# illini-robomaster/irmv_detection

Hardware: AMD Instinct MI355X
Metric: end-to-end FPS (preprocess→NMS→PnP) 640×640 YOLOv8n, 1/2/4/8 MI355X (higher is better)
Workload: dtype f16

## Files before the change

irmv_detection_amd/csrc/engine.cpp:

```cpp
#include <hip/hip_runtime.h>

#include <algorithm>
#include <chrono>
#include <cmath>
#include <cstdio>
#include <cstring>
#include <fstream>
#include <map>
#include <mutex>
#include <set>
#include <memory>
#include <string>
#include <vector>

#include "../../include/irmv_hip.h"
#include "irmv_common.hpp"
#include "numa.hpp"

using namespace irmv;

constexpr int kLightPointsCap = 4096;

static thread_local std::string g_err;
static int fail(int code, const std::string &msg)
// ... 23 lines not shown
extern "C" int irmv_device_synchronize(int device)
{
    HIP_TRY(hipSetDevice(device));
    HIP_TRY(hipDeviceSynchronize());
    return IRMV_OK;
}
extern "C" int irmv_device_count(int *count)
{
    if (!count) return fail(IRMV_ERR_ARG, "count is null");
    HIP_TRY(hipGetDeviceCount(count));
    return IRMV_OK;
}

#pragma pack(push, 1)
struct BlobHeader { char magic[4]; uint32_t version, nc, nk, reg_max, n_layers, dtype, reserved; };
struct BlobLayer { char name[32]; uint32_t cin, cout, k, stride, act, pad; uint64_t w_off, b_off; };
#pragma pack(pop)

struct LayerW {
    std::string name;
    int cin, cout, k, stride, act;
    int groups;
    const uint16_t *w;
    const float *b;
};

static float half_bits_to_float(uint16_t h)
{
    const uint32_t sign = ((uint32_t)h & 0x8000u) << 16;
    uint32_t exp = (h >> 10) & 0x1fu, man = h & 0x3ffu, x;
    if (exp == 0) {
        if (man == 0) x = sign;
        else {
            int e = -1;
            do { e++; man <<= 1; } while (!(man & 0x400u));
            x = sign | ((uint32_t)(112 - e) << 23) | ((man & 0x3ffu) << 13);
        }
    } else if (exp == 31) x = sign | 0x7f800000u | (man << 13);
    else x = sign | ((exp + 112u) << 23) | (man << 13);
    float f;
    memcpy(&f, &x, 4);
    return f;
}

static uint16_t float_to_half_bits(float f)
{
    uint32_t x;
    memcpy(&x, &f, 4);
    const uint32_t sign = (x >> 16) & 0x8000u;
    x &= 0x7fffffffu;
    if (x >= 0x7f800000u) return (uint16_t)(sign | 0x7c00u | ((x > 0x7f800000u) ? 0x200u : 0u));
    if (x >= 0x477ff000u) return (uint16_t)(sign | 0x7c00u);
    if (x < 0x33000001u) return (uint16_t)sign;
    if (x < 0x38800000u) {
        const int shift = 126 - (int)(x >> 23);
        const uint32_t man = (x & 0x7fffffu) | 0x800000u;
        uint32_t h = man >> shift;
        const uint32_t rem = man & ((1u << shift) - 1u), half = 1u << (shift - 1);
        if (rem > half || (rem == half && (h & 1u))) h++;
        return (uint16_t)(sign | h);
    }
    uint32_t h = ((x >> 23) - 112u) << 10 | ((x >> 13) & 0x3ffu);
    const uint32_t rem = x & 0x1fffu;
    if (rem > 0x1000u || (rem == 0x1000u && (h & 1u))) h++;
    return (uint16_t)(sign | h);
}

struct Tensor {
    std::string name;
    void *base = nullptr;
    size_t slot_elems = 0;
    int H = 0, W = 0, C = 0;
    bool f32 = false;
    size_t esize() const { return f32 ? 4 : 2; }
    void *slot(int s) const { return static_cast<char *>(base) + (size_t)s * slot_elems * esize(); }
};

struct SegRef { int t = -1, coff = 0, C = 0, shift = 0; };

struct TuneSwitches {
    bool untuned, verbose, warn;
    bool has_s2, has_wres;
    std::string force_s2, force_wres;
    bool force_pw, force_pwn, force_cm, force_w8, force_nt8, force_pf4;
    bool no_pw, no_pwn, no_pf2, no_pf4, no_cm, no_w8, no_nt8, no_wres, no_deep;
};

enum OpKind { OP_PRE, OP_CONV0, OP_CONV, OP_POOL, OP_NMS, OP_LIGHT, OP_FRONT, OP_C2F2, OP_C2F32, OP_DW, OP_SHUF, OP_SCAN, OP_BNECK, OP_KPT3, OP_DEMOSAIC };

struct Op {
    OpKind kind;
    std::string layer;
    ConvCfg cfg{};
    ConvCfg cfg_one{};
    char kname_one[48] = {0};
    SegRef s0, s1;
    int Hin = 0, Win = 0, Hout = 0, Wout = 0, cin = 0, cout = 0, cout_pad = 0, ksteps = 0;
    int out_t = -1, out_coff = 0, res_t = -1, res_coff = 0;
    half_t *w_packed = nullptr;
    half_t *w_k16 = nullptr;
    half_t *w_lds[4] = {nullptr, nullptr, nullptr, nullptr};
    float *bias = nullptr;
    double flops = 0, bytes = 0;
    double w_bytes = 0;
    double out_bytes = 0;
    bool pair = false;
    int level = -1;
    char kname[48] = {0};
    int sub[4] = {-1, -1, -1, -1};
    int mode = 0;
    bool shortcut = false;
    int fuse_next = -1;
    bool fused_away = false;
    int group = -1;
    int bneck = -1;
    int kpt3 = -1;
    int tune_fuse[2] = {-1, -1};
};

enum StepKind { STEP_BATCH, STEP_ONE, STEP_MATERIALIZE, STEP_POST };

struct Launch {
    int op = -1, group = -1;
    bool cfg_one = false;
    bool fused = false;
    unsigned scan = 0;
    bool keys_only = false;
    bool once = false;
    std::string name, layer;
    double flops = 0, bytes = 0, launch_bytes = 0;
};

struct GraphKey {
    int first, count;
    StepKind kind;
    bool upload;
    bool operator<(const GraphKey &o) const { return std::tie(first, count, kind, upload) < std::tie(o.first, o.count, o.kind, o.upload); }
};

struct SlotGroup {
    int first = 0, count = 0;
    hipEvent_t h2d = nullptr, out = nullptr;
    hipStream_t compute = nullptr;
    bool in_flight = false;
    bool async_up = false;
};

struct irmv_engine {
    irmv_engine_cfg cfg{};
    int nc = 0, nk = 0, A = 0, no = 0;
    int backbone = 0;
    int num_cus = 256;
    int numa_node = -1;
    bool numa_placed = false;
    struct HeadGroup { std::vector<int> members; int family = 0, nt = 1; ConvCfg cfg{}; char name[48] = {0}; };
    std::vector<HeadGroup> head_groups;
    bool post_keys_only = false;
    bool emit_scan = false;
    bool split_scan = true;
    int *cand_counts = nullptr;
    int lvl_hw[3] = {0, 0, 0}, lvl_base[3] = {0, 0, 0};
    size_t frame_bytes = 0;
    size_t src_bytes = 0;
    hipStream_t stream = nullptr;
    hipStream_t extra_streams[7] = {nullptr, nullptr, nullptr, nullptr, nullptr, nullptr, nullptr};
    int num_streams = 1;
    hipStream_t h2d_stream = nullptr;
    std::map<std::pair<int, int>, SlotGroup> groups;
// ... 1062 lines not shown
    if (cfg->point_source < 0 || cfg->point_source > 2) return fail(IRMV_ERR_ARG, "bad point_source");
    int ndev = 0;
    HIP_TRY(hipGetDeviceCount(&ndev));
    if (cfg->device < 0 || cfg->device >= ndev) return fail(IRMV_ERR_HIP, "no such HIP device");
    std::unique_ptr<irmv_engine> e(new irmv_engine);
    e->cfg = *cfg;
    {
        int cus = 0;
        if (hipDeviceGetAttribute(&cus, hipDeviceAttributeMultiprocessorCount, cfg->device) == hipSuccess && cus > 0) e->num_cus = cus;
        int node = -1;
        if (hipDeviceGetAttribute(&node, hipDeviceAttributeHostNumaId, cfg->device) == hipSuccess) e->numa_node = node;
        else (void)hipGetLastError();
    }
    int rc = load_blob(e.get());
    e->cfg.weights_path = nullptr;
    e->cfg.weights_blob = nullptr;
    if (rc) return rc;
    rc = build_engine(e.get());
    if (rc) return rc;
    rc = autotune_convs(e.get());
    if (rc) return rc;
    finalize_head_fusion(e.get());
    rc = build_head_groups(e.get());
    if (rc) return rc;
    build_step_plans(e.get());
    rc = choose_sync_launch(e.get());
    if (rc) return rc;
    *out = e.release();
    return IRMV_OK;
}

extern "C" int irmv_engine_sync_launch(const irmv_engine *e) { return e ? e->sync_launch : 0; }

extern "C" void irmv_engine_destroy(irmv_engine *e) { delete e; }
extern "C" int irmv_engine_num_slots(const irmv_engine *e) { return e ? e->cfg.num_slots : 0; }
extern "C" int irmv_engine_max_det(const irmv_engine *e) { return e ? e->cfg.max_det : 0; }
extern "C" int irmv_engine_num_streams(const irmv_engine *e) { return e ? e->num_streams : 0; }
extern "C" int irmv_engine_num_anchors(const irmv_engine *e) { return e ? e->A : 0; }
extern "C" int irmv_engine_numa_node(const irmv_engine *e) { return e ? e->numa_node : -1; }
extern "C" int irmv_engine_numa_placed(const irmv_engine *e) { return e && e->numa_placed ? 1 : 0; }

extern "C" int irmv_numa_device_node(int device, int *node)
{
    if (!node) return fail(IRMV_ERR_ARG, "node is null");
    int v = -1;
    if (hipDeviceGetAttribute(&v, hipDeviceAttributeHostNumaId, device) != hipSuccess) {
        (void)hipGetLastError();
        v = -1;
    }
    *node = v;
    return IRMV_OK;
}
extern "C" int irmv_numa_bind_thread(int node) { return numa::bind_thread_to_node(node) ? IRMV_OK : fail(IRMV_ERR_ARG, "no usable CPU on that NUMA node (or none listed in sysfs)"); }
extern "C" int irmv_numa_page_node(const void *p) { return numa::page_node(p); }
extern "C" int irmv_numa_parse_cpulist(const char *s, int *cpus, int cap)
{
    const std::vector<int> v = numa::parse_cpulist(s);
    for (size_t i = 0; i < v.size() && (int)i < cap; i++) if (cpus) cpus[i] = v[i];
    return (int)v.size();
}
extern "C" int irmv_engine_head_channels(const irmv_engine *e) { return e ? e->no : 0; }

static uint8_t *upload_dev(const irmv_engine *e) { return e->raw_dev ? e->raw_dev : e->src_dev; }

extern "C" uint8_t *irmv_engine_src_buffer(irmv_engine *e, int slot)
{
    if (!e || slot < 0 || slot >= e->cfg.num_slots) return nullptr;
    return e->src_host + (size_t)slot * e->src_bytes;
}
extern "C" void *irmv_engine_src_device_buffer(irmv_engine *e, int slot)
{
    if (!e || slot < 0 || slot >= e->cfg.num_slots) return nullptr;
    return upload_dev(e) + (size_t)slot * e->src_bytes;
}
extern "C" int irmv_engine_src_format(const irmv_engine *e) { return e ? e->cfg.src_format : -1; }
extern "C" size_t irmv_engine_src_bytes(const irmv_engine *e) { return e ? e->src_bytes : 0; }

struct TuneEntry { int mt, nt, flags, ipw; };
static bool operator==(const TuneEntry &x, const TuneEntry &y) { return x.mt == y.mt && x.nt == y.nt && x.flags == y.flags && x.ipw == y.ipw; }
static std::mutex g_tune_mu;
static std::map<std::string, TuneEntry> g_tune_cache;
static std::set<std::string> g_tune_files;

enum : int { T_LDS = 1, T_DEEP = 2, T_CT = 4, T_PW = 8, T_PF2 = 16, T_PF4 = 32, T_CM2 = 64, T_CM4 = 128, T_W8 = 256, T_WR = 512, T_PP = 1024 };
static int tile_flags(const ConvCfg &c)
{
    return (c.lds ? T_LDS : 0) | (c.deep ? T_DEEP : 0) | (c.ct ? T_CT : 0) | (c.pw ? T_PW : 0) | (c.pf2 ? T_PF2 : 0) | (c.pf4 ? T_PF4 : 0) |
           (c.cm == 2 ? T_CM2 : 0) | (c.cm == 4 ? T_CM4 : 0) | (c.w8 ? T_W8 : 0) | (c.wr ? T_WR : 0) | (c.pp ? T_PP : 0);
}
static TuneEntry tune_entry(const ConvCfg &c) { return {c.mt, c.nt, tile_flags(c), c.ipw}; }

static void tune_cache_load()
{
    const char *path = getenv("IRMV_TUNE_CACHE");
    if (!path) return;
    std::lock_guard<std::mutex> lk(g_tune_mu);
    if (!g_tune_files.insert(path).second) return;
    std::ifstream f(path);
    std::string key;
    TuneEntry t;
    while (f >> key >> t.mt >> t.nt >> t.flags >> t.ipw) g_tune_cache[key] = t;
}

static void tune_cache_save()
{
    const char *path = getenv("IRMV_TUNE_CACHE");
    if (!path) return;
    std::lock_guard<std::mutex> lk(g_tune_mu);
    std::ofstream f(path);
    for (auto &kv : g_tune_cache) f << kv.first << ' ' << kv.second.mt << ' ' << kv.second.nt << ' ' << kv.second.flags << ' ' << kv.second.ipw << '\n';
}

static int lds_index(int nt) { return nt == 8 ? 3 : (nt == 4 ? 2 : (nt == 2 ? 1 : 0)); }

static bool run_conv(const Op &op, const ConvCfg &c, const ConvArgs &a, int count, hipStream_t s)
{
    const int li = lds_index(c.nt);
    if (op.w_k16) return launch_conv_k16(a, s);
    if (c.pw) return launch_conv_pw(c, a, s);
    if (c.wr) return c.lds && op.w_lds[2] && launch_conv_wres(c.ipw, a, op.w_lds[2], count, s, c.pp);
    if (c.lds) return op.w_lds[li] && launch_conv_lds(c.stride, c.mt, c.nt, c.ipw, a, op.w_lds[li], count, s, c.pf4 ? 2 : (c.pf2 ? 1 : 0), c.cm, c.w8);
    if (c.ct) {
        if (!op.w_lds[0] || a.n2 > 0) return false;
        ConvArgs a2 = a;
        a2.w = op.w_lds[0];
        return launch_conv(c, a2, s);
    }
    return launch_conv(c, a, s);
}

static void cfg_name(const ConvCfg &c, char *buf, int n)
{
    if (c.pw) snprintf(buf, n, c.ipw > 1 ? "conv1x1s1_pw_n%d" : "conv1x1s1_pw", c.ipw);
    else if (c.wr) snprintf(buf, n, "conv3x3s1_wres%s_i%d", c.pp ? "_pp" : "", c.ipw);
    else if (c.lds && c.ipw > 1) snprintf(buf, n, "conv3x3s%d_lds_mt%d_nt%d_i%d%s%s", c.stride, c.mt, c.nt, c.ipw, c.cm ? "_cm" : (c.pf4 ? "_p4" : (c.pf2 ? "_p2" : "")), c.w8 ? "_w8" : "");
    else if (c.lds) snprintf(buf, n, "conv3x3s%d_lds_mt%d_nt%d%s%s", c.stride, c.mt, c.nt, c.pf4 ? "_p4" : (c.pf2 ? "_p2" : ""), c.w8 ? "_w8" : "");
    else conv_cfg_name(c, buf, n);
}

static void fill_conv_args(const irmv_engine *e, const Op &op, int first, int count, ConvArgs &a, bool fused = false);

static ConvCfg tile_cfg(const ConvCfg &base, int mt, int nt, int flags, int ipw)
{
    ConvCfg c = base;
    c.mt = mt; c.nt = nt; c.ipw = ipw;
    c.lds = flags & T_LDS; c.deep = flags & T_DEEP; c.ct = flags & T_CT; c.pw = flags & T_PW; c.pf2 = flags & T_PF2; c.pf4 = flags & T_PF4;
    c.cm = (flags & T_CM2) ? 2 : ((flags & T_CM4) ? 4 : 0); c.w8 = flags & T_W8; c.wr = flags & T_WR; c.pp = flags & T_PP;
    return c;
}

static TuneSwitches tune_switches()
{
    auto on = [](const char *name) { return getenv(name) != nullptr; };
    const char *at = getenv("IRMV_AUTOTUNE"), *nd = getenv("IRMV_NO_DEEP");
    TuneSwitches s;
    s.untuned = at && at[0] == '0'; s.verbose = on("IRMV_AUTOTUNE_VERBOSE"); s.warn = on("IRMV_TUNE_WARN");
    const char *s2 = getenv("IRMV_FORCE_S2"), *wres = getenv("IRMV_FORCE_WRES");
    s.has_s2 = s2 != nullptr; s.force_s2 = s2 ? s2 : "";
    s.has_wres = wres != nullptr; s.force_wres = wres ? wres : "";
    s.force_pw = on("IRMV_FORCE_PW"); s.force_pwn = on("IRMV_FORCE_PWN"); s.force_cm = on("IRMV_FORCE_CM");
    s.force_w8 = on("IRMV_FORCE_W8"); s.force_nt8 = on("IRMV_FORCE_NT8"); s.force_pf4 = on("IRMV_FORCE_PF4");
    s.no_pw = on("IRMV_NO_PW"); s.no_pwn = on("IRMV_NO_PWN"); s.no_pf2 = on("IRMV_NO_PF2"); s.no_pf4 = on("IRMV_NO_PF4");
    s.no_cm = on("IRMV_NO_CM"); s.no_w8 = on("IRMV_NO_W8"); s.no_nt8 = on("IRMV_NO_NT8"); s.no_wres = on("IRMV_NO_WRES");
    s.no_deep = nd && nd[0] == '1';
    return s;
}

struct TuneCand { ConvCfg c; bool forced; };

static std::vector<TuneCand> tune_candidates(const Op &op, const ConvArgs &a, int count, bool want_fuse, bool lds_ok, const TuneSwitches &sw, int num_cus)
{
    std::vector<TuneCand> v;
    const bool s2 = sw.has_s2 && lds_ok && op.cfg.stride == 2;
    auto add = [&](const ConvCfg &c, bool forced = false) {
        if (op.cout_pad % (16 * c.nt) != 0) return;
        if (s2 && !forced && sw.force_s2 != (c.lds ? "lds" : (c.deep ? "deep" : "ct"))) return;
        if (c.wr ? !(op.w_lds[2] && conv_wres_bytes(a, c.stride, c.pp) > 0)
                 : c.lds && !(op.w_lds[lds_index(c.nt)] && conv_lds_bytes(a, c.stride, c.mt, c.nt, nullptr, c.w8) > 0)) return;
        v.push_back({c, forced});
    };
    const int ipw_max = lds_ok ? std::min(4, count) : 1;
    for (int mt = 1; mt <= 4; mt *= 2)
        for (int nt = 1; nt <= 4; nt *= 2)
            for (int ipw = 1; ipw <= ipw_max; ipw *= 2)
                if (!want_fuse || nt == 4) add(tile_cfg(op.cfg, mt, nt, lds_ok ? T_LDS : 0, ipw));
    if (lds_ok && !want_fuse && !sw.no_pf2)
        for (int nt = 1; nt <= 4; nt *= 2)
            for (int ipw = 1; ipw <= ipw_max; ipw *= 2) add(tile_cfg(op.cfg, 1, nt, T_LDS | T_PF2, ipw));
    if (lds_ok && !want_fuse && !sw.no_pf4 && op.cin >= 128 && op.w_lds[0]) add(tile_cfg(op.cfg, 1, 1, T_LDS | T_PF4, 1), sw.force_pf4);
    if (lds_ok && !sw.no_cm)
        for (int mt = 1; mt <= 2; mt *= 2)
            for (int ipw = 2; ipw <= std::min(mt == 1 ? 4 : 2, count); ipw *= 2)
                if (!(want_fuse && mt == 1 && ipw == 2)) add(tile_cfg(op.cfg, mt, 4, T_LDS | (ipw == 2 ? T_CM2 : T_CM4), ipw), sw.force_cm);
    if (lds_ok && op.cfg.stride == 2 && !want_fuse && !sw.no_w8)
        for (int mt = 1; mt <= 2; mt *= 2)
            for (int ipw = 1; ipw <= ipw_max; ipw *= 2)
                for (int cmv = 0; cmv < 2; cmv++)
                    if (!cmv || (mt == 2 && ipw == 2) || (mt == 1 && ipw == 4)) add(tile_cfg(op.cfg, mt, 4, T_LDS | T_W8 | (cmv ? (ipw == 2 ? T_CM2 : T_CM4) : 0), ipw), sw.force_w8);
    if (lds_ok && op.cfg.stride == 2 && !want_fuse && !sw.no_w8 && !sw.no_nt8)
        for (int ipw = 1; ipw <= ipw_max; ipw *= 2)
            for (int cmv = 0; cmv < 2; cmv++)
                if (!cmv || ipw == 2) add(tile_cfg(op.cfg, 1, 8, T_LDS | T_W8 | (cmv ? T_CM2 : 0), ipw), sw.force_nt8);
    if (lds_ok && count >= 2 && !sw.no_wres)
        for (int ppv = 0; ppv < 2; ppv++) {
            const int wgt = conv_wres_tiles(a, op.cfg.stride, ppv != 0);
            if (wgt <= 0) continue;
            int ipw1 = 1;
            while (ipw1 < count && (long)wgt * ((count + ipw1 - 1) / ipw1) > num_cus) ipw1++;
            const int cand[3] = {ipw1, (ipw1 + 1) / 2, std::min(count, 2 * ipw1)};
            for (int k = 0; k < 3; k++)
                if (k == 0 || (cand[k] != cand[0] && (k == 1 || cand[2] != cand[1]))) add(tile_cfg(op.cfg, 2, 4, T_LDS | T_WR | (ppv ? T_PP : 0), cand[k]));
        }
    if (sw.has_wres && lds_ok && count >= 2) {
        const int n = atoi(sw.force_wres.c_str());
        for (int ppv = 0; ppv <= (n > 0 ? 1 : 0); ppv++) add(tile_cfg(op.cfg, 2, 4, T_LDS | T_WR | (ppv ? T_PP : 0), std::max(1, std::min(count, n < 0 ? -n : n))), true);
    }
    if (conv_pw_eligible(op.cfg, a) && !sw.no_pw) {
        add(tile_cfg(op.cfg, 2, 4, T_PW, 1), sw.force_pw);
        for (int nbw = 2; nbw <= 4 && !sw.no_pwn; nbw *= 2)
            if (conv_pw_lds_bytes(a, nbw)) add(tile_cfg(op.cfg, 2, 4, T_PW, nbw), sw.force_pwn);
    }
    if (lds_ok && !want_fuse && op.w_lds[0] && op.cfg.stride == 2 && !op.cfg.cin16)
        for (int mt = 1; mt <= 4; mt *= 2)
            for (int nt = 1; nt <= 4; nt *= 2) add(tile_cfg(op.cfg, mt, nt, T_CT, 1));
    if ((count == 1 || op.cfg.ks == 1) && !want_fuse && !sw.no_deep && !op.cfg.cin16 && !op.cfg.out_f32 && op.cfg.act == 1 && (!lds_ok || op.w_lds[0])) {
        const int tiles[4][2] = {{1, 1}, {2, 1}, {1, 2}, {1, 4}};
        for (auto &t : tiles) add(tile_cfg(op.cfg, t[0], t[1], T_DEEP | (lds_ok ? T_CT : 0), 1));
    }
    return v;
}

struct ConvView { ConvArgs a; bool want_fuse, lds_ok; };
static ConvView conv_view(const irmv_engine *e, const Op &op, int first, int count)
{
    ConvView v;
    const bool fuse_k16 = op.fuse_next >= 0 && op.cfg.cin16;
    v.want_fuse = op.fuse_next >= 0 && !fuse_k16;
    fill_conv_args(e, op, first, count, v.a, v.want_fuse || fuse_k16);
    if (v.want_fuse) {
        bool f_ok = false;
        for (int mt = 1; mt <= 4 && !f_ok; mt *= 2) f_ok = op.w_lds[2] && conv_lds_bytes(v.a, op.cfg.stride, mt, 4, nullptr) > 0;
        if (!f_ok) {
            v.want_fuse = false;
            fill_conv_args(e, op, first, count, v.a, false);
        }
    }
    v.lds_ok = false;
    if (op.cfg.ks == 3 && op.cfg.act == 1 && !op.cfg.out_f32)
        for (int mt = 1; mt <= 4 && !v.lds_ok; mt *= 2)
            for (int nt = 1; nt <= 4 && !v.lds_ok; nt *= 2) v.lds_ok = op.w_lds[lds_index(nt)] && conv_lds_bytes(v.a, op.cfg.stride, mt, nt, nullptr) > 0;
    return v;
}

static int autotune_convs(irmv_engine *e)
{
    const TuneSwitches sw = tune_switches();
    e->tune_sw = sw;
    tune_cache_load();
    hipEvent_t ea, eb;
    HIP_TRY(hipEventCreate(&ea));
    HIP_TRY(hipEventCreate(&eb));
    const int counts[2] = {stream_share(e, e->cfg.num_slots), 1};
    for (Op &op : e->ops) {
        if (op.kind != OP_CONV) continue;
        for (int pass = 0; pass < (counts[0] > 1 ? 2 : 1); pass++) {
            const int count = counts[pass];
            op.tune_fuse[pass] = op.fuse_next;
            const ConvView v = conv_view(e, op, 0, count);
            if (!v.want_fuse && !op.cfg.cin16) op.fuse_next = -1;
            const ConvArgs &a = v.a;
            const bool want_fuse = v.want_fuse, lds_ok = v.lds_ok;
            char key[160];
            snprintf(key, sizeof key, "gfx950.t5|%d.%d.%d.%d.%d.%d|%dx%d>%dx%d|c%d.%d.%d.%d>%d|ld%d.%d.%d|n%d|%d", op.cfg.ks, op.cfg.stride,
                     (int)op.cfg.cin16, op.cfg.act, (int)op.cfg.out_f32, (int)lds_ok, a.Hin, a.Win, a.Hout, a.Wout, a.s0.C, a.s1.C, a.s0.shift,
                     a.s1.shift, a.cout_pad, a.s0.ld, a.s1.ld, a.out_ld, count, (a.res ? 1 : 0) + 2 * a.n2);
            const std::vector<TuneCand> cands = tune_candidates(op, a, count, want_fuse, lds_ok, sw, e->num_cus);
            const bool forced = (sw.has_s2 && lds_ok && op.cfg.stride == 2) || std::any_of(cands.begin(), cands.end(), [](const TuneCand &k) { return k.forced; });
            ConvCfg best_cfg = pass == 0 ? op.cfg : op.cfg_one;
            bool have_hit = false;
            if (!forced && !sw.untuned && !sw.verbose) {
                std::lock_guard<std::mutex> lk(g_tune_mu);
                auto hit = g_tune_cache.find(key);
                if (hit != g_tune_cache.end()) {
                    const TuneEntry &h = hit->second;
                    auto it = std::find_if(cands.begin(), cands.end(), [&](const TuneCand &k) { return tune_entry(k.c) == h; });
                    if (it != cands.end()) { best_cfg = it->c; have_hit = true; }
                    else if (sw.warn) fprintf(stderr, "[autotune] cached tile for %s rejected (mt %d nt %d lds %d ipw %d): re-tuning\n", key, h.mt, h.nt, h.flags & 1, h.ipw);
                }
            }
            float best = 1e30f;
            for (size_t i = 0; i < cands.size() && !have_hit; i++) {
                const ConvCfg &c = cands[i].c;
                if (cands[i].forced) {
                    if (run_conv(op, c, a, count, e->stream)) { best = 0.f; best_cfg = c; }
                    continue;
                }
                if (sw.untuned && best < 1e29f) continue;
                bool ok = true;
                for (int r = 0; r < 2 && ok; r++) ok = run_conv(op, c, a, count, e->stream);
                if (!ok) continue;
                if (sw.untuned) { best = 0.f; best_cfg = c; continue; }
                float ms = 1e30f;
                for (int rep = 0; rep < 3; rep++) {
// ... 1165 lines not shown
```

irmv_detection_amd/csrc/irmv_common.hpp:

```cpp
#pragma once

#include <hip/hip_runtime.h>

#include <cstdint>
#include <cstdlib>

namespace irmv {

typedef _Float16 half_t;
typedef _Float16 half8 __attribute__((ext_vector_type(8)));
typedef _Float16 half4 __attribute__((ext_vector_type(4)));
typedef float f32x4 __attribute__((ext_vector_type(4)));

constexpr float kActScale = 1.44269504088896341f;
constexpr float kActUnscale = 0.693147180559945309f;
typedef unsigned int u32x4_t __attribute__((ext_vector_type(4)));
__device__ __forceinline__ float silu_rcp(float y) { return __builtin_amdgcn_rcpf(1.0f + __builtin_amdgcn_exp2f(-y)); }
__device__ __forceinline__ unsigned int silu_pack2(float y0, float y1)
{
    const float r0 = silu_rcp(y0), r1 = silu_rcp(y1);
    unsigned int o;
    asm("v_fma_mixlo_f16 %0, %1, %2, 0" : "=v"(o) : "v"(y0), "v"(r0));
    asm("v_fma_mixhi_f16 %0, %1, %2, 0" : "+v"(o) : "v"(y1), "v"(r1));
    return o;
// ... 170 lines not shown
    int cat_ld;
    half_t *out;
    int out_ld;
    int H, W, tiles_x, tiles_y;
    const half_t *w_m1, *w_m2;
    const float *b_m1, *b_m2;
    const half_t *w_cv2;
    const float *b_cv2;
};
size_t bneck64_lds_bytes(int mode, int ks2);
bool launch_bneck64(int mode, int ks2, bool shortcut, const BneckArgs &a, int batch, hipStream_t s);

constexpr int kKpt3Tile = 10;
struct Kpt3Args {
    const half_t *x;
    int x_ld;
    int H, W, tiles_x, tiles_y;
    const half_t *w1;
    const float *b1;
    const half_t *w2;
    const float *b2;
    const half_t *w3;
    const float *b3;
    float *out;
    int out_ld;
};
bool kpt3_eligible(int cin);
bool launch_kpt3(const Kpt3Args &a, int cin, int batch, hipStream_t s);

struct ConvArgs {
    ConvSeg s0, s1;
    int Hin, Win;
    int Hout, Wout;
    int M;
    int Cin;
    const half_t *w;
    const float *bias;
    void *out;
    int out_ld;
    const half_t *res;
    int res_ld;
    int cout_pad;
    int ksteps;
    int pair;
    const half_t *w2;
    const float *bias2;
    float *out2;
    int out2_ld, n2;
    unsigned long long *scan_keys;
    int *scan_counts;
    float scan_thr;
    int scan_nc, scan_abase, scan_key_cap;
};

constexpr int kMultiMax = 6;
struct LdsMember {
    ConvArgs a;
    const half_t *wl;
    int tiles_x, tiles_y, twc_log2, patch_bytes, batch, tile2d;
    int gx, gy;
};
struct LdsMultiArgs {
    int n;
    int start[kMultiMax + 1];
    LdsMember m[kMultiMax];
};
struct DirectMultiArgs {
    int n;
    int start[kMultiMax + 1], gx[kMultiMax], gy[kMultiMax];
    ConvArgs a[kMultiMax];
};

struct ConvCfg {
    int ks, stride, mt, nt; bool cin16; int act; bool out_f32; bool lds; int ipw;
    bool deep;
    bool ct;
    bool pw;
    bool pf2;
    bool pf4;
    bool w8;
    int cm;
    bool wr;
    bool pp;
};
bool launch_conv(const ConvCfg &cfg, const ConvArgs &a, hipStream_t s);
const char *conv_cfg_name(const ConvCfg &cfg, char *buf, int n);
bool conv_pw_eligible(const ConvCfg &cfg, const ConvArgs &a);
bool launch_conv_lds_multi(int nt, const ConvArgs *a, const half_t *const *wl, int n, int batch, hipStream_t s);
bool launch_conv_direct_multi(const ConvCfg &cfg, const ConvArgs *a, int n, hipStream_t s);
bool launch_conv_k16(const ConvArgs &a, hipStream_t s);
bool launch_conv_pw(const ConvCfg &cfg, const ConvArgs &a, hipStream_t s);
size_t conv_pw_lds_bytes(const ConvArgs &a, int nbw);
size_t conv_lds_bytes(const ConvArgs &a, int stride, int mt, int nt, int *patch_rows_max, bool w8 = false);
size_t conv_wres_bytes(const ConvArgs &a, int stride, bool pp);
int conv_wres_tiles(const ConvArgs &a, int stride, bool pp);
bool launch_conv_wres(int ipw, const ConvArgs &a, const half_t *wl, int batch, hipStream_t s, bool pp);
bool launch_conv_lds(int stride, int mt, int nt, int ipw, const ConvArgs &a, const half_t *wl, int batch, hipStream_t s, int pf2 = 0, int cm = 0, bool w8 = false);

void launch_sppf_pool(half_t *buf, int batch, int H, int W, int C, hipStream_t s);

struct DevDet {
    float box_net[4];
    float xyxy[4];
    float score;
    int32_t cls, anchor, pnp_ok;
    float kpts_net[8];
    float kpts[8];
    double rvec[3], tvec[3], quat[4];
    int32_t armor_valid;
    int32_t armor_size;
    int32_t n_lights;
    int32_t pad_;
};
struct DevFrameOut { int32_t num_dets, n_candidates, overflow, pad; };

struct PnpConst {
    double fx, fy, cx, cy, k1, k2, p1, p2, k3;
    double hy[2], hz[2];
};

struct PostArgs {
    const float *head_all;
    int slots_total, first;
    float *boxes;
    unsigned long long *keys;
    int key_cap;
    DevDet *dets;
    DevFrameOut *fout;
    int net, A, nc, nk;
    float logit_thr, iou_thr;
    int max_det, pre_nms_cap;
    float scale_x, scale_y, off_x, off_y;
    int armor_size;
    const PnpConst *pnp;
    long long *dbg;
    int keys_only;
    int prefilter;
    int classwalk;
    int *counts;
};
void launch_nms_pnp(const PostArgs &a, int batch, hipStream_t s);
constexpr int kScanBlocks = 16;
void launch_scan_decode(const PostArgs &a, int batch, hipStream_t s);
constexpr int kLightLdsPoints = 256;
constexpr int kLightLdsImage = 40 * 1024;
constexpr int kLightMaxContours = 1024;

struct LightArgs {
    const uint8_t *frames;
    size_t frame_bytes;
    int cols, rows, rotate180;
    DevDet *dets;
    int max_det;
    const int *num_dets;
    int num_dets_stride, n_boxes;
    const float *boxes;
    signed char *labels;
    size_t label_pool;
    short *points;
    int points_cap;
    short *hulls;
    int binary_threshold;
    float light_min_ratio, light_max_ratio, light_max_angle;
    double min_small_cd, max_small_cd, min_large_cd, max_large_cd;
    const PnpConst *pnp;
    int pnp_armor_size;
};
void launch_light_extract(const LightArgs &a, int n_boxes_max, int batch, hipStream_t s);

void launch_pnp_only(const PnpConst &c, const float *pts, int n, int armor_size, double *rvec, double *tvec,
                     int32_t *ok, hipStream_t s);

}
```

irmv_detection_amd/csrc/k_conv.hip:

```cpp
#include "irmv_common.hpp"

#include <cstdio>
#include <mutex>
#include <type_traits>

namespace irmv {

template <int MT, int NT>
struct PrefetchDepth { static constexpr int value = (MT * NT >= 8) ? 2 : ((MT * NT >= 4) ? 3 : 4); };
template <int MT, int NT>
struct DeepPrefetchDepth { static constexpr int value = (MT + NT <= 2) ? 12 : ((MT + NT <= 3) ? 10 : 6); };


template <int KS, int STRIDE, int MT, int NT, bool CIN16, int ACT, bool OUT_F32, bool CT = false, bool DEEP = false>
__device__ __forceinline__ void conv_mfma_body(const ConvArgs &a, int wg_x, int wg_y, int grid_x, int grid_y)
{
    constexpr int PAD = KS / 2;
    constexpr int PF = DEEP ? DeepPrefetchDepth<MT, NT>::value : PrefetchDepth<MT, NT>::value;
    static_assert(!CT || (KS == 3 && !CIN16), "chunk-major order is the 3x3 LDS family's");
    const int lane = threadIdx.x & 63, wave = threadIdx.x >> 6;
    const int g = lane >> 4, r = lane & 15;
    const int bx = wg_x, by = wg_y;
    (void)grid_x; (void)grid_y;
    const int tile0 = (bx * 4 + wave) * MT;
// ... 495 lines not shown
                p1[mt] = a.s1.p + (size_t)mm * a.s1.ld + 8 * g - a.s0.C;
            } else {
                const int b = mm / HWo, rem = mm - b * HWo;
                const int oy = rem / a.Wout, ox = rem - oy * a.Wout;
                p0[mt] = a.s0.p + ((size_t)(b * H0 + (oy >> a.s0.shift)) * W0 + (ox >> a.s0.shift)) * a.s0.ld + 8 * g;
                p1[mt] = a.s1.p + ((size_t)(b * H1 + (oy >> a.s1.shift)) * W1 + (ox >> a.s1.shift)) * a.s1.ld + 8 * g - a.s0.C;
            }
        }
    };
    auto load_b = [&](int mt, int ks) -> half8 {
        const int c = ks * 32;
        return *reinterpret_cast<const half8 *>((c < a.s0.C ? p0[mt] : p1[mt]) + c);
    };
    half8 B[MT][KS];
    tile_ptrs(u0);
#pragma unroll
    for (int ks = 0; ks < KS; ks++)
#pragma unroll
        for (int mt = 0; mt < MT; mt++) B[mt][ks] = load_b(mt, ks);
#pragma unroll
    for (int i = 0; i < WPT; i++) {
        const int e = tid + i * NTH;
        if (e < WALL) s_w[e] = wreg[i];
    }
    __syncthreads();
    half_t *out = static_cast<half_t *>(a.out);
    auto run_tile = [&](auto mta_c, auto pre_c, int ub) {
        constexpr int MTA = decltype(mta_c)::value;
        constexpr bool PRE = decltype(pre_c)::value;
        size_t m_cur[MTA];
        bool mv_cur[MTA];
#pragma unroll
        for (int mt = 0; mt < MTA; mt++) { m_cur[mt] = (size_t)(ub + mt) * 16 + r; mv_cur[mt] = mv[mt]; }
        if constexpr (PRE) tile_ptrs(ub + MT);
#pragma unroll
        for (int nb = 0; nb < NBW; nb++) {
            const half8 *s_wb = s_w + nb * (NT * KS * 64) + lane;
            f32x4 acc[MTA][NT];
#pragma unroll
            for (int nt = 0; nt < NT; nt++) {
                const f32x4 b = *reinterpret_cast<const f32x4 *>(s_bias + nb * 64 + (nt >> 1) * 32 + g * 8 + (nt & 1) * 4);
#pragma unroll
                for (int mt = 0; mt < MTA; mt++) acc[mt][nt] = b;
            }
            half8 A[2][NT];
#pragma unroll
            for (int nt = 0; nt < NT; nt++) A[0][nt] = s_wb[(nt * KS) * 64];
#pragma unroll
            for (int ks = 0; ks < KS; ks++) {
                if (ks + 1 < KS) {
#pragma unroll
                    for (int nt = 0; nt < NT; nt++) A[(ks + 1) & 1][nt] = s_wb[(nt * KS + ks + 1) * 64];
                }
#pragma unroll
                for (int mt = 0; mt < MTA; mt++) {
#pragma unroll
                    for (int nt = 0; nt < NT; nt++) acc[mt][nt] = __builtin_amdgcn_mfma_f32_16x16x32_f16(A[ks & 1][nt], B[mt][ks], acc[mt][nt], 0, 0, 0);
                    if constexpr (PRE) if (nb == NBW - 1) B[mt][ks] = load_b(mt, ks);
                }
                __builtin_amdgcn_sched_barrier(0);
            }
#pragma unroll
            for (int mt = 0; mt < MTA; mt++) {
                if (!mv_cur[mt]) continue;
#pragma unroll
                for (int u = 0; u < 2; u++) {
                    float vals[8];
#pragma unroll
                    for (int i = 0; i < 4; i++) {
                        vals[i] = acc[mt][2 * u][i];
                        vals[4 + i] = acc[mt][2 * u + 1][i];
                    }
                    const half8 o = silu_pack8(vals[0], vals[1], vals[2], vals[3], vals[4], vals[5], vals[6], vals[7]);
                    *reinterpret_cast<half8 *>(out + m_cur[mt] * a.out_ld + ((nblk0 + nb) * 2 + u) * 32 + g * 8) = o;
                }
            }
        }
    };
    int ub = u0;
    for (; ub + MT <= u1; ub += MT) run_tile(std::integral_constant<int, MT>{}, std::true_type{}, ub);
    if (ub < u1) run_tile(std::integral_constant<int, 1>{}, std::false_type{}, ub);
}

bool conv_pw_eligible(const ConvCfg &c, const ConvArgs &a)
{
    return c.ks == 1 && c.stride == 1 && c.act == 1 && !c.out_f32 && !c.cin16 && a.pair && a.cout_pad % 64 == 0 && a.Cin % 32 == 0 && a.s0.C % 32 == 0 &&
           (a.ksteps == 4 || a.ksteps == 6 || a.ksteps == 8 || a.ksteps == 12 || a.ksteps == 16) && a.res == nullptr && a.n2 == 0;
}

size_t conv_pw_lds_bytes(const ConvArgs &a, int nbw)
{
    if (!(nbw == 2 || nbw == 4) || a.cout_pad % (64 * nbw) != 0) return 0;
    const int ks = a.ksteps;
    if (!(ks == 4 || ks == 6 || ks == 8 || ks == 12 || ks == 16) || nbw * ks > 32) return 0;
    return (size_t)nbw * 4 * ks * 1024 + (size_t)nbw * 64 * 4;
}

bool launch_conv_pw(const ConvCfg &c, const ConvArgs &a, hipStream_t s)
{
    if (!conv_pw_eligible(c, a)) return false;
    const int tiles_total = (a.M + 31) / 32, nblocks = a.cout_pad / 64;
    if (c.ipw > 1) {
        const int nbw = c.ipw;
        const size_t lds = conv_pw_lds_bytes(a, nbw);
        if (!lds) return false;
        const int groups = nblocks / nbw;
        const int units = (a.M + 15) / 16;
#define IRMV_PWN(KS_, NBW_)                                                                                          \
        if (a.ksteps == KS_ && nbw == NBW_) {                                                                          \
            static unsigned long long attr_done = 0;                                                                   \
                                    \
            static int per_cu[64], cus[64];                                                                            \
            int dev = 0;                                                                                               \
            (void)hipGetDevice(&dev);                                                                                  \
            dev &= 63;                                                                                                 \
            once_per_device(attr_done, [lds, dev] {                                                                    \
                (void)hipFuncSetAttribute(reinterpret_cast<const void *>(conv1x1_pwn_kernel<KS_, NBW_>), hipFuncAttributeMaxDynamicSharedMemorySize, 160 * 1024); \
                int nb = 0, nc = 0;                                                                                    \
                per_cu[dev] = 1; cus[dev] = 256;                                                                       \
                if (hipOccupancyMaxActiveBlocksPerMultiprocessor(&nb, reinterpret_cast<const void *>(conv1x1_pwn_kernel<KS_, NBW_>), 512, lds) == hipSuccess && nb >= 1) per_cu[dev] = nb > 2 ? 2 : nb; \
                if (hipDeviceGetAttribute(&nc, hipDeviceAttributeMultiprocessorCount, dev) == hipSuccess && nc > 0) cus[dev] = nc; \
            });                                                                                                        \
            int wg = (cus[dev] * per_cu[dev] + groups - 1) / groups;                    \
            if (wg > (units + 7) / 8) wg = (units + 7) / 8;               \
            if (wg < 1) wg = 1;                                                                                        \
            hipLaunchKernelGGL((conv1x1_pwn_kernel<KS_, NBW_>), dim3(wg, groups), dim3(512), lds, s, a, wg);           \
            return true;                                                                                               \
        }
        IRMV_PWN(4, 2) IRMV_PWN(6, 2) IRMV_PWN(8, 2) IRMV_PWN(12, 2) IRMV_PWN(16, 2) IRMV_PWN(4, 4) IRMV_PWN(6, 4) IRMV_PWN(8, 4)
#undef IRMV_PWN
        return false;
    }
    int wg = (tiles_total + 3) / 4;
    const int cap = (512 + nblocks - 1) / nblocks;
    if (wg > cap) wg = cap;
    if (wg < 1) wg = 1;
#define IRMV_PW(KS_)                                                                                               \
    if (a.ksteps == KS_) {                                                                                          \
        static unsigned long long attr_done = 0;                                                                    \
        once_per_device(attr_done, [] {                                                                             \
            (void)hipFuncSetAttribute(reinterpret_cast<const void *>(conv1x1_pw_kernel<KS_>), hipFuncAttributeMaxDynamicSharedMemorySize, 96 * 1024); \
        });                                                                                                         \
        hipLaunchKernelGGL((conv1x1_pw_kernel<KS_>), dim3(wg, nblocks), dim3(256), (size_t)4 * KS_ * 1024, s, a, tiles_total, wg);            \
        return true;                                                                                                \
    }
    IRMV_PW(4) IRMV_PW(6) IRMV_PW(8) IRMV_PW(12) IRMV_PW(16)
#undef IRMV_PW
    return false;
}

constexpr int lds_pmax(int stride, int mt, bool tile2d, int wr = 0, int pf = 0)
{
    return pf == 2 ? (stride == 1 ? 4 : 8) : (wr ? 4 : ((tile2d && stride == 1) ? (mt == 4 ? 8 : 4) : 12));
}

#ifndef IRMV_LDS_WAVES
#define IRMV_LDS_WAVES 2
#endif
template <int STRIDE, int MT, int NT, bool TILE2D, int N2, int PF = 0, int CM = 0, int NWV = 4, int WR = 0, bool PP = false>
__device__ __forceinline__ void conv3x3_lds_body(const ConvArgs &a, const half_t *wl, int tiles_x, int tiles_y, int twc_log2, int a_patch_bytes, int ipw, int batch,
                                                 int wg_x, int wg_y, int grid_x, int grid_y, int stagger = 0)
{
    extern __shared__ __attribute__((aligned(16))) unsigned char smem[];
    const int lane = threadIdx.x & 63, wave = threadIdx.x >> 6, tid = threadIdx.x;
    constexpr bool PF2 = PF != 0;
    constexpr int NPF = PF == 2 ? 4 : (PF == 1 ? 2 : 1);
    constexpr int NTH = 64 * NWV;
    static_assert(!PP || (WR > 0 && NWV % 2 == 0), "ping-pong groups share resident weights");
    constexpr int NWP = PP ? NWV / 2 : NWV;
    constexpr int NTP = 64 * NWP;
    const int sub = PP ? wave / NWP : 0, wv = wave - sub * NWP, tidp = tid - sub * NTP;
    const int g = lane >> 4, r = lane & 15;
    const int bx = wg_x, by = wg_y;
    (void)grid_x; (void)grid_y;
    const int wg_tiles = PP ? (tiles_x * tiles_y + 1) / 2 : tiles_x * tiles_y;
    const int grp = bx / wg_tiles;
    int tile = PP ? 2 * (bx - grp * wg_tiles) + sub : bx - grp * wg_tiles;
    const bool active = tile < tiles_x * tiles_y;
    if (!active) tile = 0;
    const int img = grp * ipw, nimg = min(ipw, batch - img);
    const int nblk = by;
    const int HWo = a.Hout * a.Wout;
    int PW, PR, iy_base, ix_base;
// ... 847 lines not shown
```

Before: 62000.

## Add upsample-aware 1x1 pointwise conv kernel reusing low-res source across 2x2 outputs

Adds a specialized 1x1 conv kernel for concat inputs where one segment is a nearest-upsampled (shift=1) tensor. Each work unit computes four output pixels of a 2x2 block together, sharing the low-res partial sum (bias plus upsampled-segment contribution) across them. This removes redundant reads and MFMA work on the upsampled channels. It is added as an autotune candidate, enabled by default and switchable off with an env var, at the cost of more register pressure and extra tuning candidates.

```diff
diff --git a/irmv_detection_amd/csrc/engine.cpp b/irmv_detection_amd/csrc/engine.cpp
--- a/irmv_detection_amd/csrc/engine.cpp
+++ b/irmv_detection_amd/csrc/engine.cpp
@@ -129,8 +129,9 @@
     bool untuned, verbose, warn;
     bool has_s2, has_wres;
     std::string force_s2, force_wres;
-    bool force_pw, force_pwn, force_cm, force_w8, force_nt8, force_pf4;
+    bool force_pw, force_pwn, force_cm, force_w8, force_nt8, force_pf4, force_pwup;
     bool no_pw, no_pwn, no_pf2, no_pf4, no_cm, no_w8, no_nt8, no_wres, no_deep;
+    bool upsample_src;
 };
 
 enum OpKind { OP_PRE, OP_CONV0, OP_CONV, OP_POOL, OP_NMS, OP_LIGHT, OP_FRONT, OP_C2F2, OP_C2F32, OP_DW, OP_SHUF, OP_SCAN, OP_BNECK, OP_KPT3, OP_DEMOSAIC };
@@ -1359,11 +1360,11 @@
 static std::map<std::string, TuneEntry> g_tune_cache;
 static std::set<std::string> g_tune_files;
 
-enum : int { T_LDS = 1, T_DEEP = 2, T_CT = 4, T_PW = 8, T_PF2 = 16, T_PF4 = 32, T_CM2 = 64, T_CM4 = 128, T_W8 = 256, T_WR = 512, T_PP = 1024 };
+enum : int { T_LDS = 1, T_DEEP = 2, T_CT = 4, T_PW = 8, T_PF2 = 16, T_PF4 = 32, T_CM2 = 64, T_CM4 = 128, T_W8 = 256, T_WR = 512, T_PP = 1024, T_UP = 2048 };
 static int tile_flags(const ConvCfg &c)
 {
     return (c.lds ? T_LDS : 0) | (c.deep ? T_DEEP : 0) | (c.ct ? T_CT : 0) | (c.pw ? T_PW : 0) | (c.pf2 ? T_PF2 : 0) | (c.pf4 ? T_PF4 : 0) |
-           (c.cm == 2 ? T_CM2 : 0) | (c.cm == 4 ? T_CM4 : 0) | (c.w8 ? T_W8 : 0) | (c.wr ? T_WR : 0) | (c.pp ? T_PP : 0);
+           (c.cm == 2 ? T_CM2 : 0) | (c.cm == 4 ? T_CM4 : 0) | (c.w8 ? T_W8 : 0) | (c.wr ? T_WR : 0) | (c.pp ? T_PP : 0) | (c.up ? T_UP : 0);
 }
 static TuneEntry tune_entry(const ConvCfg &c) { return {c.mt, c.nt, tile_flags(c), c.ipw}; }
 
@@ -1408,7 +1409,8 @@
 
 static void cfg_name(const ConvCfg &c, char *buf, int n)
 {
-    if (c.pw) snprintf(buf, n, c.ipw > 1 ? "conv1x1s1_pw_n%d" : "conv1x1s1_pw", c.ipw);
+    if (c.pw && c.up) snprintf(buf, n, "conv1x1s1_pw_up_n%d", c.ipw);
+    else if (c.pw) snprintf(buf, n, c.ipw > 1 ? "conv1x1s1_pw_n%d" : "conv1x1s1_pw", c.ipw);
     else if (c.wr) snprintf(buf, n, "conv3x3s1_wres%s_i%d", c.pp ? "_pp" : "", c.ipw);
     else if (c.lds && c.ipw > 1) snprintf(buf, n, "conv3x3s%d_lds_mt%d_nt%d_i%d%s%s", c.stride, c.mt, c.nt, c.ipw, c.cm ? "_cm" : (c.pf4 ? "_p4" : (c.pf2 ? "_p2" : "")), c.w8 ? "_w8" : "");
     else if (c.lds) snprintf(buf, n, "conv3x3s%d_lds_mt%d_nt%d%s%s", c.stride, c.mt, c.nt, c.pf4 ? "_p4" : (c.pf2 ? "_p2" : ""), c.w8 ? "_w8" : "");
@@ -1422,7 +1424,7 @@
     ConvCfg c = base;
     c.mt = mt; c.nt = nt; c.ipw = ipw;
     c.lds = flags & T_LDS; c.deep = flags & T_DEEP; c.ct = flags & T_CT; c.pw = flags & T_PW; c.pf2 = flags & T_PF2; c.pf4 = flags & T_PF4;
-    c.cm = (flags & T_CM2) ? 2 : ((flags & T_CM4) ? 4 : 0); c.w8 = flags & T_W8; c.wr = flags & T_WR; c.pp = flags & T_PP;
+    c.cm = (flags & T_CM2) ? 2 : ((flags & T_CM4) ? 4 : 0); c.w8 = flags & T_W8; c.wr = flags & T_WR; c.pp = flags & T_PP; c.up = flags & T_UP;
     return c;
 }
 
@@ -1437,6 +1439,8 @@
     s.has_wres = wres != nullptr; s.force_wres = wres ? wres : "";
     s.force_pw = on("IRMV_FORCE_PW"); s.force_pwn = on("IRMV_FORCE_PWN"); s.force_cm = on("IRMV_FORCE_CM");
     s.force_w8 = on("IRMV_FORCE_W8"); s.force_nt8 = on("IRMV_FORCE_NT8"); s.force_pf4 = on("IRMV_FORCE_PF4");
+    s.force_pwup = on("IRMV_FORCE_PWUP");
+    { const char *up = getenv("IRMV_UPSAMPLE_SRC"); s.upsample_src = !(up && up[0] == '0'); }
     s.no_pw = on("IRMV_NO_PW"); s.no_pwn = on("IRMV_NO_PWN"); s.no_pf2 = on("IRMV_NO_PF2"); s.no_pf4 = on("IRMV_NO_PF4");
     s.no_cm = on("IRMV_NO_CM"); s.no_w8 = on("IRMV_NO_W8"); s.no_nt8 = on("IRMV_NO_NT8"); s.no_wres = on("IRMV_NO_WRES");
     s.no_deep = nd && nd[0] == '1';
@@ -1496,6 +1500,8 @@
         add(tile_cfg(op.cfg, 2, 4, T_PW, 1), sw.force_pw);
         for (int nbw = 2; nbw <= 4 && !sw.no_pwn; nbw *= 2)
             if (conv_pw_lds_bytes(a, nbw)) add(tile_cfg(op.cfg, 2, 4, T_PW, nbw), sw.force_pwn);
+        for (int nbw = 1; nbw <= 2 && sw.upsample_src; nbw *= 2)
+            if (conv_pwup_lds_bytes(a, nbw)) add(tile_cfg(op.cfg, 1, 4, T_PW | T_UP, nbw), sw.force_pwup);
     }
     if (lds_ok && !want_fuse && op.w_lds[0] && op.cfg.stride == 2 && !op.cfg.cin16)
         for (int mt = 1; mt <= 4; mt *= 2)
diff --git a/irmv_detection_amd/csrc/irmv_common.hpp b/irmv_detection_amd/csrc/irmv_common.hpp
--- a/irmv_detection_amd/csrc/irmv_common.hpp
+++ b/irmv_detection_amd/csrc/irmv_common.hpp
@@ -276,6 +276,7 @@
     int cm;
     bool wr;
     bool pp;
+    bool up;
 };
 bool launch_conv(const ConvCfg &cfg, const ConvArgs &a, hipStream_t s);
 const char *conv_cfg_name(const ConvCfg &cfg, char *buf, int n);
@@ -285,6 +286,7 @@
 bool launch_conv_k16(const ConvArgs &a, hipStream_t s);
 bool launch_conv_pw(const ConvCfg &cfg, const ConvArgs &a, hipStream_t s);
 size_t conv_pw_lds_bytes(const ConvArgs &a, int nbw);
+size_t conv_pwup_lds_bytes(const ConvArgs &a, int nbw);
 size_t conv_lds_bytes(const ConvArgs &a, int stride, int mt, int nt, int *patch_rows_max, bool w8 = false);
 size_t conv_wres_bytes(const ConvArgs &a, int stride, bool pp);
 int conv_wres_tiles(const ConvArgs &a, int stride, bool pp);
diff --git a/irmv_detection_amd/csrc/k_conv.hip b/irmv_detection_amd/csrc/k_conv.hip
--- a/irmv_detection_amd/csrc/k_conv.hip
+++ b/irmv_detection_amd/csrc/k_conv.hip
@@ -601,6 +601,133 @@
     if (ub < u1) run_tile(std::integral_constant<int, 1>{}, std::false_type{}, ub);
 }
 
+template <int KS0, int KS1, int NBW>
+__global__ __launch_bounds__(512) void conv1x1_pwup_kernel(ConvArgs a, int wg_per_group)
+{
+    constexpr int KS = KS0 + KS1, NT = 4, NTH = 512;
+    extern __shared__ __attribute__((aligned(16))) unsigned char smem[];
+    half8 *s_w = reinterpret_cast<half8 *>(smem);
+    float *s_bias = reinterpret_cast<float *>(smem + (size_t)NBW * NT * KS * 1024);
+    const int tid = threadIdx.x, lane = tid & 63, wave = tid >> 6;
+    const int g = lane >> 4, r = lane & 15;
+    const int nblk0 = blockIdx.y * NBW;
+    constexpr int WALL = NBW * NT * KS * 64, WPT = (WALL + NTH - 1) / NTH;
+    half8 wreg[WPT];
+    {
+        const half8 *wsrc = reinterpret_cast<const half8 *>(a.w) + (size_t)nblk0 * NT * KS * 64;
+#pragma unroll
+        for (int i = 0; i < WPT; i++) {
+            const int e = tid + i * NTH;
+            wreg[i] = wsrc[e < WALL ? e : WALL - 1];
+        }
+    }
+    if (tid < NBW * 64) s_bias[tid] = a.bias[nblk0 * 64 + tid];
+    const int W0 = a.Wout >> 1, HW0 = (a.Hout >> 1) * W0, Ms = a.M >> 2;
+    const int units = (Ms + 15) >> 4, nw = wg_per_group * 8, wv = blockIdx.x * 8 + wave;
+    const int u0 = (int)((long long)wv * units / nw), u1 = (int)((long long)(wv + 1) * units / nw);
+    auto c_off = [&](int c) -> int { return (c >> 1) * a.Wout + (c & 1); };
+    const half_t *p0, *p1;
+    size_t m00;
+    bool mv;
+    auto unit_ptrs = [&](int ub) {
+        const int sp = ub * 16 + r;
+        mv = ub < u1 && sp < Ms;
+        const int ss = mv ? sp : 0;
+        const int b = ss / HW0, rem = ss - b * HW0;
+        const int sy = rem / W0, sx = rem - sy * W0;
+        m00 = ((size_t)b * a.Hout + 2 * sy) * a.Wout + 2 * sx;
+        p0 = a.s0.p + (size_t)ss * a.s0.ld + 8 * g;
+        p1 = a.s1.p + m00 * a.s1.ld + 8 * g;
+    };
+    auto load0 = [&](int ks) -> half8 { return *reinterpret_cast<const half8 *>(p0 + ks * 32); };
+    auto load1 = [&](int c, int ks) -> half8 { return *reinterpret_cast<const half8 *>(p1 + (size_t)c_off(c) * a.s1.ld + ks * 32); };
+    half8 B0[KS0], B1[4][KS1];
+    unit_ptrs(u0);
+#pragma unroll
+    for (int ks = 0; ks < KS0; ks++) B0[ks] = load0(ks);
+#pragma unroll
+    for (int c = 0; c < 4; c++)
+#pragma unroll
+        for (int ks = 0; ks < KS1; ks++) B1[c][ks] = load1(c, ks);
+#pragma unroll
+    for (int i = 0; i < WPT; i++) {
+        const int e = tid + i * NTH;
+        if (e < WALL) s_w[e] = wreg[i];
+    }
+    __syncthreads();
+    half_t *out = static_cast<half_t *>(a.out);
+    auto run_unit = [&](auto pre_c, int ub) {
+        constexpr bool PRE = decltype(pre_c)::value;
+        const size_t m_cur = m00;
+        const bool mv_cur = mv;
+        if constexpr (PRE) unit_ptrs(ub + 1);
+#pragma unroll
+        for (int nb = 0; nb < NBW; nb++) {
+            const half8 *s_wb = s_w + nb * (NT * KS * 64) + lane;
+            const bool last = nb == NBW - 1;
+            f32x4 acc0[NT];
+#pragma unroll
+            for (int nt = 0; nt < NT; nt++) acc0[nt] = *reinterpret_cast<const f32x4 *>(s_bias + nb * 64 + (nt >> 1) * 32 + g * 8 + (nt & 1) * 4);
+            half8 A[2][NT];
+#pragma unroll
+            for (int nt = 0; nt < NT; nt++) A[0][nt] = s_wb[(nt * KS) * 64];
+#pragma unroll
+            for (int ks = 0; ks < KS0; ks++) {
+                const int kn = ks + 1;
+#pragma unroll
+                for (int nt = 0; nt < NT; nt++) A[kn & 1][nt] = s_wb[(nt * KS + kn) * 64];
+#pragma unroll
+                for (int nt = 0; nt < NT; nt++) acc0[nt] = __builtin_amdgcn_mfma_f32_16x16x32_f16(A[ks & 1][nt], B0[ks], acc0[nt], 0, 0, 0);
+                if constexpr (PRE) if (last) B0[ks] = load0(ks);
+                __builtin_amdgcn_sched_barrier(0);
+            }
+#pragma unroll
+            for (int cp = 0; cp < 2; cp++) {
+                f32x4 acc[2][NT];
+#pragma unroll
+                for (int h = 0; h < 2; h++)
+#pragma unroll
+                    for (int nt = 0; nt < NT; nt++) acc[h][nt] = acc0[nt];
+#pragma unroll
+                for (int ks = 0; ks < KS1; ks++) {
+                    const int st = KS0 + cp * KS1 + ks;
+                    if (ks + 1 < KS1 || cp == 0) {
+                        const int kn = ks + 1 < KS1 ? KS0 + ks + 1 : KS0;
+#pragma unroll
+                        for (int nt = 0; nt < NT; nt++) A[(st + 1) & 1][nt] = s_wb[(nt * KS + kn) * 64];
+                    }
+#pragma unroll
+                    for (int h = 0; h < 2; h++) {
+#pragma unroll
+                        for (int nt = 0; nt < NT; nt++) acc[h][nt] = __builtin_amdgcn_mfma_f32_16x16x32_f16(A[st & 1][nt], B1[2 * cp + h][ks], acc[h][nt], 0, 0, 0);
+                        if constexpr (PRE) if (last) B1[2 * cp + h][ks] = load1(2 * cp + h, ks);
+                    }
+                    __builtin_amdgcn_sched_barrier(0);
+                }
+                if (!mv_cur) continue;
+#pragma unroll
+                for (int h = 0; h < 2; h++) {
+                    const size_t m = m_cur + c_off(2 * cp + h);
+#pragma unroll
+                    for (int u = 0; u < 2; u++) {
+                        float vals[8];
+#pragma unroll
+                        for (int i = 0; i < 4; i++) {
+                            vals[i] = acc[h][2 * u][i];
+                            vals[4 + i] = acc[h][2 * u + 1][i];
+                        }
+                        const half8 o = silu_pack8(vals[0], vals[1], vals[2], vals[3], vals[4], vals[5], vals[6], vals[7]);
+                        *reinterpret_cast<half8 *>(out + m * a.out_ld + ((nblk0 + nb) * 2 + u) * 32 + g * 8) = o;
+                    }
+                }
+            }
+        }
+    };
+    int ub = u0;
+    for (; ub + 1 < u1; ub++) run_unit(std::true_type{}, ub);
+    if (ub < u1) run_unit(std::false_type{}, ub);
+}
+
 bool conv_pw_eligible(const ConvCfg &c, const ConvArgs &a)
 {
     return c.ks == 1 && c.stride == 1 && c.act == 1 && !c.out_f32 && !c.cin16 && a.pair && a.cout_pad % 64 == 0 && a.Cin % 32 == 0 && a.s0.C % 32 == 0 &&
@@ -615,9 +742,51 @@
     return (size_t)nbw * 4 * ks * 1024 + (size_t)nbw * 64 * 4;
 }
 
+size_t conv_pwup_lds_bytes(const ConvArgs &a, int nbw)
+{
+    if (a.s0.shift != 1 || a.s1.shift != 0 || a.s1.C <= 0 || a.s0.C % 32 != 0 || a.s1.C % 32 != 0) return 0;
+    if (a.Hout != a.Hin || a.Wout != a.Win || a.Hout % 2 != 0 || a.Wout % 2 != 0 || a.M % 4 != 0) return 0;
+    if (!(nbw == 1 || nbw == 2) || a.cout_pad % (64 * nbw) != 0) return 0;
+    const int k0 = a.s0.C / 32, k1 = a.s1.C / 32;
+    if (!((k0 == 8 && k1 == 4) || (k0 == 4 && k1 == 2 && nbw == 1))) return 0;
+    return (size_t)nbw * 4 * (k0 + k1) * 1024 + (size_t)nbw * 64 * 4;
+}
+
+static bool launch_conv_pwup(const ConvArgs &a, int nbw, hipStream_t s)
+{
+    const size_t lds = conv_pwup_lds_bytes(a, nbw);
+    if (!lds) return false;
+    const int groups = a.cout_pad / 64 / nbw;
+    const int units = (a.M / 4 + 15) / 16;
+#define IRMV_PWUP(KS0_, KS1_, NBW_)                                                                                  \
+    if (a.s0.C == KS0_ * 32 && a.s1.C == KS1_ * 32 && nbw == NBW_) {                                                 \
+        static unsigned long long attr_done = 0;                                                                     \
+        static int per_cu[64], cus[64];                                        \
+        int dev = 0;                                                                                                 \
+        (void)hipGetDevice(&dev);                                                                                    \
+        dev &= 63;                                                                                                   \
+        once_per_device(attr_done, [lds, dev] {                                                                      \
+            (void)hipFuncSetAttribute(reinterpret_cast<const void *>(conv1x1_pwup_kernel<KS0_, KS1_, NBW_>), hipFuncAttributeMaxDynamicSharedMemorySize, 160 * 1024); \
+            int nb = 0, nc = 0;                                                                                      \
+            per_cu[dev] = 1; cus[dev] = 256;                                                                         \
+            if (hipOccupancyMaxActiveBlocksPerMultiprocessor(&nb, reinterpret_cast<const void *>(conv1x1_pwup_kernel<KS0_, KS1_, NBW_>), 512, lds) == hipSuccess && nb >= 1) per_cu[dev] = nb > 2 ? 2 : nb; \
+            if (hipDeviceGetAttribute(&nc, hipDeviceAttributeMultiprocessorCount, dev) == hipSuccess && nc > 0) cus[dev] = nc; \
+        });                                                                                                          \
+        int wg = (cus[dev] * per_cu[dev] + groups - 1) / groups;                                                     \
+        if (wg > (units + 7) / 8) wg = (units + 7) / 8;                                                              \
+        if (wg < 1) wg = 1;                                                                                          \
+        hipLaunchKernelGGL((conv1x1_pwup_kernel<KS0_, KS1_, NBW_>), dim3(wg, groups), dim3(512), lds, s, a, wg);     \
+        return true;                                                                                                 \
+    }
+    IRMV_PWUP(8, 4, 1) IRMV_PWUP(8, 4, 2) IRMV_PWUP(4, 2, 1)
+#undef IRMV_PWUP
+    return false;
+}
+
 bool launch_conv_pw(const ConvCfg &c, const ConvArgs &a, hipStream_t s)
 {
     if (!conv_pw_eligible(c, a)) return false;
+    if (c.up) return launch_conv_pwup(a, c.ipw, s);
     const int tiles_total = (a.M + 31) / 32, nblocks = a.cout_pad / 64;
     if (c.ipw > 1) {
         const int nbw = c.ipw;
```

Result: no change. 61970, median of 6 (-0.0%).
